# Excalibur-SLE/spmv

Hardware: AMD Instinct MI355X
Metric: fp64 CG iters/sec (SpMV effective GB/s vs HBM roofline) (higher is better)
Workload: dtype f64

## Files before the change

spmv_amd/csrc/hip/common.h:

```cpp
#pragma once

#include <mutex>
#include <vector>

#include <hip/hip_runtime.h>

#include <cstdint>
#include <cstdlib>

#include "spmv_hip.h"

struct spmv_hip_ctx {
  int device = 0;
  int num_cus = 0;
  hipStream_t stream = nullptr;
  int dot_blocks = 0;
  int64_t blas1_nt_min_elems = (int64_t)1 << 24;
  int64_t lx_min_nnz = (int64_t)1 << 20;
  int64_t lx_max_x_bytes = INT64_MAX;
  int lx_dma = 1;
  int lx_codes = 1;
  int lx_narrow_values = 1;
  int lx_ring = 1;
  int release_csr = 0;
  int64_t xw_min_nnz = (int64_t)1 << 20;
  int64_t xw_min_x_bytes = (int64_t)128 << 20;
  int xw_probe = 1;
  int csr_in_place = 0;
  int64_t lat_min_nnz = (int64_t)1 << 20;
  int bake_general = 1;
  int wdia_half = 1;
  int const_diagonals = 1;
  int const_tile = 4;
  int64_t sj_min_nnz = (int64_t)1 << 20;
  int sj_max_chunks = 432;
  int sj_wpb = 0;
  int sj_unit = 0;
  int sj_sigma = 1;
// ... 113 lines not shown
```

spmv_amd/csrc/hip/csr_plan.h:

```cpp
#pragma once

#include "common.h"

#include <chrono>
#include <cstdio>

constexpr int kRows = kBlock;

typedef double f64x2 __attribute__((ext_vector_type(2)));
typedef float f32x4 __attribute__((ext_vector_type(4)));
typedef int i32x2 __attribute__((ext_vector_type(2)));
typedef int i32x4 __attribute__((ext_vector_type(4)));

template <typename T>
struct VecOf;
template <>
struct VecOf<double> {
  static constexpr int V = 2;
  using val_t = f64x2;
  using col_t = i32x2;
};
template <>
struct VecOf<float> {
  static constexpr int V = 4;
// ... 109 lines not shown
}
__host__ __device__ constexpr bool lx_ring_fits(int cnt)
{
  return cnt > 0 && cnt + 3 <= kLxwRingVcap
         && lx_ring_code_bytes(cnt) <= kLxwRingCodeMax;
}
constexpr int kLxwDescStartBits = 11;
constexpr int kLxwDescStartMask = (1 << kLxwDescStartBits) - 1;
constexpr int kLxwDescMaxLen = (1 << (16 - kLxwDescStartBits)) - 1;
static_assert(kLxwRingVcap <= kLxwDescStartMask + 1, "a row's start needs more bits");
constexpr int kLxwDescPad = 1024 - kRows * 2;
__host__ __device__ constexpr int64_t lx_rowdesc_bytes(int64_t num_row_blocks)
{
  return num_row_blocks * (kRows * 2) + kLxwDescPad;
}
constexpr int kXwMaxWin = 8;
constexpr int kXwFirst0 = kLxwPieces0 + kLxwMaxPieces;
constexpr int kXwDelta0 = kXwFirst0 + kXwMaxWin;
constexpr int kXwRec = 36;

constexpr int kLatMaxOff = 8;
constexpr int kLatRec = 12;
constexpr int kWdiaMaxOff = 32;

struct PlanTrace {
  bool on;
  std::chrono::steady_clock::time_point t0;
  const char* who;
  explicit PlanTrace(const char* w)
      : on(getenv("SPMV_PLAN_TRACE") != nullptr), t0(std::chrono::steady_clock::now()),
// ... 183 lines not shown
  int lxw_max_cnt = 0;
  int lxw_max_pieces = 0;
  int lxw_blocks_per_cu = 0;
  int lxw_grid_cap = 0;
  uint8_t* lx_code = nullptr;
  int lx4 = 0;
  int lx4_blocks = 0;
  int lx4_lut = 1;
  int lx_ring_blocks = 0;
  uint16_t* lx_rowdesc = nullptr;
  int lx_ring_pwr = 0;
  int lx_ring = 1;
  float* lx_val32 = nullptr;
  const void* lx32_values0 = nullptr;
  int lx_v32 = 0;
  int32_t* xw_rec = nullptr;
  int xw = 0;
  int xw_staged = 0;
  int xw_max_cnt = 0, xw_max_pieces = 0;
  struct XwProbe* xw_probe = nullptr;
  int32_t* lat_tab = nullptr;
  uint8_t* lat_mask = nullptr;
  int lat = 0;
  int lat_blocks = 0;
  int lat_blocks_per_cu = 4;
  int lat_xcd_group = 0;
  int lat_chain = 1;

  int lattice_d1 = 0, lattice_d2 = 0;

// ... 23 lines not shown
  int use_xw = 1;
  hipEvent_t ev[4][2] = {};
  float us_xw = 0.f, us_gather = 0.f;
};

int spmv_rowblock_grid(const spmv_hip_csr_plan* pl);
bool spmv_released_launch_ok(const spmv_hip_csr_plan* pl, const void* values,
                             const void* in, const void* diagonal, int elem_bytes);
int spmv_build_row_list(spmv_hip_csr_plan* pl, const int32_t* rowptr);
void spmv_free_lx(spmv_hip_csr_plan* pl);
void spmv_free_xw(spmv_hip_csr_plan* pl);
int spmv_build_lx(spmv_hip_csr_plan* pl, const int32_t* rowptr, const int32_t* colind);
int spmv_lx32_bake(spmv_hip_csr_plan* pl, const double* values, bool may_alloc,
                   hipStream_t st);
void spmv_lx32_free(spmv_hip_csr_plan* pl);
int spmv_build_xw_and_walk(spmv_hip_csr_plan* pl, const int32_t* rowptr,
                           const int32_t* colind);
bool spmv_xw_applies(const spmv_hip_csr_plan* pl);
void xw_probe_free(spmv_hip_csr_plan* pl);
void xw_probe_drop_events(XwProbe* pb);
int spmv_plan_owned_mask(const spmv_hip_csr_plan* pl);
int spmv_run_symmetric_f64(const spmv_hip_csr_plan* pl, hipStream_t st,
                           const int32_t* rowptr, const int32_t* colind,
                           const double* values, const double* diagonal,
                           double alpha, const double* in, double beta,
                           double* out, DotOut dot);
int spmv_run_symmetric_f32(const spmv_hip_csr_plan* pl, hipStream_t st,
                           const int32_t* rowptr, const int32_t* colind,
                           const float* values, const float* diagonal,
                           float alpha, const float* in, float beta,
// ... 43 lines not shown
                         double* out, DotOut dot);
int spmv_sdia_run_f64(const spmv_hip_csr_plan* pl, hipStream_t st, double alpha,
                      const double* in, double beta, double* out, DotOut dot);
int spmv_sdia_run_f32(const spmv_hip_csr_plan* pl, hipStream_t st, float alpha,
                      const float* in, float beta, float* out);
int spmv_lxw_grid(const spmv_hip_csr_plan* pl, int elem_bytes);
bool spmv_lxw_ring_ok(const spmv_hip_csr_plan* pl, bool forced);
int spmv_lxw_run_f64(const spmv_hip_csr_plan* pl, hipStream_t st,
                     const int32_t* rowptr, const int32_t* colind,
                     const double* values, double alpha, const double* in,
                     double beta, double* out, DotOut dot);
int spmv_lxw_run_f32f64(const spmv_hip_csr_plan* pl, hipStream_t st,
                        const int32_t* rowptr, const int32_t* colind,
                        const float* values, double alpha, const double* in,
                        double beta, double* out, DotOut dot);
int spmv_xw_grid(const spmv_hip_csr_plan* pl, int elem_bytes);
int spmv_xw_run_f64(const spmv_hip_csr_plan* pl, hipStream_t st,
                    const int32_t* rowptr, const int32_t* colind,
                    const double* values, double alpha, const double* in,
                    double beta, double* out, DotOut dot);
int spmv_xw_run_f32(const spmv_hip_csr_plan* pl, hipStream_t st,
                    const int32_t* rowptr, const int32_t* colind,
                    const float* values, float alpha, const float* in,
                    float beta, float* out);
int spmv_lxw_run_f32(const spmv_hip_csr_plan* pl, hipStream_t st,
                     const int32_t* rowptr, const int32_t* colind,
                     const float* values, float alpha, const float* in,
                     float beta, float* out);
void spmv_wdia_free(spmv_hip_csr_plan* pl);
int spmv_wdia_walk_build(spmv_hip_csr_plan* pl, int segments, bool force);
// ... 56 lines not shown
```

spmv_amd/csrc/hip/runtime.hip:

```cpp
#include "common.h"

#include <cstdio>
#include <cstring>
#include <new>

bool spmv_ctx_watch(spmv_hip_ctx* ctx, const int32_t* word, bool add)
{
  std::lock_guard<std::mutex> lock(ctx->watched_mutex);
  auto& ws = ctx->watched;
  if (add) {
    try {
      ws.push_back(word);
    } catch (...) {
      return false;
    }
    return true;
  }
  for (size_t i = 0; i < ws.size(); ++i)
    if (ws[i] == word) {
      ws[i] = ws.back();
      ws.pop_back();
      break;
    }
  return true;
// ... 131 lines not shown
    *value = ctx->xw_min_nnz;
  else if (!strcmp(key, "xw_min_x_bytes"))
    *value = ctx->xw_min_x_bytes;
  else if (!strcmp(key, "xw_probe"))
    *value = ctx->xw_probe;
  else if (!strcmp(key, "csr_in_place"))
    *value = ctx->csr_in_place;
  else if (!strcmp(key, "lx_min_nnz"))
    *value = ctx->lx_min_nnz;
  else if (!strcmp(key, "lat_min_nnz"))
    *value = ctx->lat_min_nnz;
  else if (!strcmp(key, "lx_narrow_values"))
    *value = ctx->lx_narrow_values;
  else if (!strcmp(key, "lx_ring"))
    *value = ctx->lx_ring;
  else if (!strcmp(key, "sj_min_nnz"))
    *value = ctx->sj_min_nnz;
  else
    return SPMV_HIP_EINVAL;
  return SPMV_HIP_OK;
}

int spmv_hip_ctx_set_option(spmv_hip_ctx* ctx, const char* key, int64_t value)
{
  SPMV_REQUIRE(ctx && key);
  if (!strcmp(key, "blas1_nt_min_elems")) {
    SPMV_REQUIRE(value >= 0);
    ctx->blas1_nt_min_elems = value;
    return SPMV_HIP_OK;
  }
// ... 48 lines not shown
    return SPMV_HIP_OK;
  }
  if (!strcmp(key, "lx_codes")) {
    SPMV_REQUIRE(value == 0 || value == 1);
    ctx->lx_codes = (int)value;
    return SPMV_HIP_OK;
  }
  if (!strcmp(key, "lx_narrow_values")) {
    SPMV_REQUIRE(value == 0 || value == 1);
    ctx->lx_narrow_values = (int)value;
    return SPMV_HIP_OK;
  }
  if (!strcmp(key, "lx_ring")) {
    SPMV_REQUIRE(value >= 0 && value <= 2);
    ctx->lx_ring = (int)value;
    return SPMV_HIP_OK;
  }
  if (!strcmp(key, "poisson_stencil")) {
    SPMV_REQUIRE(value == 7 || value == 27);
    ctx->poisson_stencil = (int)value;
    return SPMV_HIP_OK;
  }
  if (!strcmp(key, "const_diagonals")) {
    SPMV_REQUIRE(value == 0 || value == 1);
    ctx->const_diagonals = (int)value;
    return SPMV_HIP_OK;
  }
  if (!strcmp(key, "const_tile")) {
    SPMV_REQUIRE(value == 1 || value == 2 || value == 4);
    ctx->const_tile = (int)value;
// ... 272 lines not shown
```

spmv_amd/csrc/hip/spmv_csr.hip:

```cpp
#include "csr_plan.h"

#include <cstring>
#include <new>

namespace
{

template <typename TV, typename T, int CH, bool NT, bool ALIGNED, bool DOT,
          bool XCD>
__global__ __launch_bounds__(kBlock) void csr_rowblock_kernel(
    int32_t num_rows, int64_t nnz, const int32_t* __restrict__ rowptr,
    const int32_t* __restrict__ colind, const TV* __restrict__ values, T alpha,
    const T* __restrict__ in, T beta, T* __restrict__ out,
    DotOut dot, RowBlockOrder ord)
{
  constexpr int V = VecOf<TV>::V;
  constexpr int TILE = kBlock * CH * V;
  using val_t = typename VecOf<TV>::val_t;
  using col_t = typename VecOf<TV>::col_t;
  typedef T prod_t __attribute__((ext_vector_type(V)));

  __shared__ __attribute__((aligned(32))) T s_prod[TILE];
  __shared__ int32_t s_rowptr[kRows + 1];
  __shared__ double s_red[kBlock / 64];
// ... 507 lines not shown
    if constexpr (sizeof(T) == 8)
      return spmv_sjds_run_f64(pl, st, alpha, in, beta, out,
                               DOT ? dot : DotOut());
    else
      return spmv_sjds_run_f32(pl, st, alpha, in, beta, out);
  }
  if (pl->lat && aligned16(values)) {
    if constexpr (sizeof(T) == 8)
      return spmv_lat_run_f64(pl, st, rowptr, values, alpha, in, beta, out,
                              DOT ? dot : DotOut());
    else
      return spmv_lat_run_f32(pl, st, rowptr, values, alpha, in, beta, out);
  }
  if (pl->lx && pl->lxw && pl->lxw_rec && al && aligned16(in)) {
    if constexpr (sizeof(T) == 8) {
      if (pl->lx_v32 && pl->lx_val32 && values == pl->lx32_values0)
        return spmv_lxw_run_f32f64(pl, st, rowptr, colind, pl->lx_val32, alpha,
                                   in, beta, out, DOT ? dot : DotOut());
      return spmv_lxw_run_f64(pl, st, rowptr, colind, values, alpha, in, beta,
                              out, DOT ? dot : DotOut());
    } else
      return spmv_lxw_run_f32(pl, st, rowptr, colind, values, alpha, in, beta,
                              out);
  }
  if (pl->lx && al && aligned16(in)) {
    LxView lx{pl->lx_lidx, pl->lx_tab};
    RowBlockOrder lx_ord = pl->row_block_order(nrb);
    if (pl->zwalk && pl->zw_table && pl->zw_grid == grid) {
      lx_ord.table = pl->zw_table;
      lx_ord.num_slots = pl->zw_slots;
// ... 352 lines not shown
```

spmv_amd/csrc/hip/spmv_csr_forms.hip:

```cpp
#include "csr_plan.h"

#include <hipcub/hipcub.hpp>

#include <algorithm>
#include <chrono>
#include <cstring>
#include <new>
#include <utility>
#include <vector>

#include "plan_scratch.h"

namespace
{

template <int ITEMS>
__global__ __launch_bounds__(kBlock) void lx_build_kernel(
    int32_t num_rows, int32_t num_cols, const int32_t* __restrict__ rowptr,
    const int32_t* __restrict__ colind, uint16_t* __restrict__ lidx,
    int32_t* __restrict__ tab, int num_row_blocks, int end_bit, int align,
    int pad, int cap, int32_t* __restrict__ wrec, int32_t* __restrict__ stat,
    int xw)
{
  using Sort = hipcub::BlockRadixSort<int32_t, kBlock, ITEMS, int32_t>;
// ... 334 lines not shown
  pl->num_listed = count;
  return SPMV_HIP_OK;
}

void spmv_free_lx(spmv_hip_csr_plan* pl)
{
  plan_drop(pl->lx_lidx);
  plan_drop(pl->lx_tab);
  plan_drop(pl->lxw_rec);
  plan_drop(pl->lx_code);
  plan_drop(pl->lx_rowdesc);
  pl->lx = pl->lx_staged = pl->lx_blocks = 0;
  pl->lxw = pl->lxw_max_cnt = pl->lxw_max_pieces = 0;
  pl->lx4 = pl->lx4_blocks = pl->lx_ring_blocks = 0;
  spmv_lx32_free(pl);
}

static int build_lx_rowdesc(spmv_hip_csr_plan* pl, const int32_t* rowptr, int nrb,
                            hipStream_t st)
{
  const size_t bytes = (size_t)lx_rowdesc_bytes(nrb);
  hipError_t e = spmv_plan_malloc(&pl->lx_rowdesc, bytes);
  if (e == hipSuccess)
    e = hipMemsetAsync(pl->lx_rowdesc, 0, bytes, st);
  if (e == hipSuccess) {
    int grid = pl->ctx->num_cus * 8;
    grid = grid > nrb ? nrb : grid;
    hipLaunchKernelGGL(lx_rowdesc_kernel, dim3(grid), dim3(kBlock), 0, st,
                       pl->num_rows, rowptr, pl->lxw_rec, pl->lx_rowdesc, nrb);
    e = hipGetLastError();
// ... 144 lines not shown
    e = hipGetLastError();
    if (e == hipSuccess)
      e = hipStreamSynchronize(st);
    if (e == hipSuccess) {
      pl->lx32_values0 = values;
      pl->lx_v32 = 1;
      pl->plan_us += (int)std::chrono::duration_cast<std::chrono::microseconds>(
                         std::chrono::steady_clock::now() - t0)
                         .count();
      return SPMV_HIP_OK;
    }
  }
  spmv_lx32_free(pl);
  if (e == hipErrorOutOfMemory)
    (void)hipGetLastError();
  pl->plan_us += (int)std::chrono::duration_cast<std::chrono::microseconds>(
                     std::chrono::steady_clock::now() - t0)
                     .count();
  return e == hipSuccess || e == hipErrorOutOfMemory ? SPMV_HIP_OK
                                                     : static_cast<int>(e);
}

void spmv_free_xw(spmv_hip_csr_plan* pl)
{
  plan_drop(pl->xw_rec);
  pl->xw = pl->xw_staged = pl->xw_max_cnt = pl->xw_max_pieces = 0;
  xw_probe_free(pl);
}

struct RowBlockEntries {
// ... 405 lines not shown
```

spmv_amd/csrc/hip/spmv_csr_plan.hip:

```cpp
#include "csr_plan.h"

#include <hipcub/hipcub.hpp>

#include <algorithm>
#include <chrono>
#include <cstring>
#include <new>
#include <utility>
#include <vector>

#include "plan_scratch.h"

thread_local int64_t spmv_plan_mem_ns = 0;
thread_local int64_t spmv_plan_live_allocs = 0;

extern "C" int spmv_hip_plan_live_allocations(int64_t* count)
{
  SPMV_REQUIRE(count != nullptr);
  *count = spmv_plan_live_allocs;
  return SPMV_HIP_OK;
}

namespace
{
// ... 82 lines not shown
  SPMV_REQUIRE(ctx && plan && num_rows >= 0 && num_cols >= 0
               && num_non_zeros >= 0);
  SPMV_REQUIRE(num_non_zeros == 0 || (rowptr && colind));
  if (num_non_zeros > 0) {
    SPMV_SET_DEVICE(ctx);
    SPMV_CHECK_HIP(hipStreamSynchronize(spmv_stream(ctx, nullptr)));
  }
  const auto t_begin = std::chrono::steady_clock::now();
  if (num_non_zeros > INT32_MAX)
    return SPMV_HIP_ERANGE;
  spmv_hip_csr_plan* pl = new (std::nothrow) spmv_hip_csr_plan;
  if (!pl)
    return SPMV_HIP_ENOMEM;
  pl->ctx = ctx;
  pl->lx_ring = ctx->lx_ring;
  MemClock mem_clock(pl);
  pl->num_rows = num_rows;
  pl->num_cols = num_cols;
  pl->nnz = num_non_zeros;
  pl->symmetric = symmetric != 0;
  pl->rowptr0 = rowptr;
  pl->colind0 = colind;
  const double avg = num_rows > 0 ? (double)num_non_zeros / num_rows : 0.0;
  if (algo == SPMV_HIP_ALGO_AUTO) {
    if (!symmetric && num_non_zeros > 0 && num_non_zeros * 4 < num_rows)
      algo = SPMV_HIP_ALGO_ROWLIST;
    else
      algo = (avg <= 64.0 || num_non_zeros >= ctx->sj_min_nnz)
                 ? SPMV_HIP_ALGO_ROWBLOCK
                 : SPMV_HIP_ALGO_VECTOR;
// ... 145 lines not shown
        return rx;
      plan->plan_us += (int)std::chrono::duration_cast<std::chrono::microseconds>(
                           std::chrono::steady_clock::now() - t0)
                           .count();
    }
  }
  if (plan->symmetric && (values == nullptr ? plan->sjt != nullptr
                                            : rc == SPMV_HIP_ENOTSUP)) {
    const int rj = sym_sj_bake<double>(ctx, plan, values, diagonal, st);
    rc = values == nullptr ? (rj != SPMV_HIP_OK ? rj : rc) : rj;
  }
  const int rn = spmv_lx32_bake(plan, rc == SPMV_HIP_ENOTSUP ? values : nullptr,
                                !plan->no_new_forms, st);
  if (rn != SPMV_HIP_OK)
    return rn;
  return rc;
}

int spmv_hip_csr_plan_bake_values_f32(spmv_hip_ctx* ctx, spmv_hip_csr_plan* plan,
                                      const float* values, const float* diagonal,
                                      void* stream)
{
  SPMV_SET_DEVICE(ctx);
  SPMV_REQUIRE(plan && plan->ctx == ctx);
  MemClock mem_clock(plan);
  SPMV_REQUIRE(!plan->released);
  hipStream_t st = spmv_stream(ctx, stream);
  if (values)
    SPMV_CHECK_HIP(hipStreamSynchronize(st));
  int rc = spmv_sdia_bake_f32(plan, values, diagonal, st);
// ... 26 lines not shown
      const auto t0 = std::chrono::steady_clock::now();
      const int rx = spmv_build_xw_and_walk(plan, plan->rowptr0, plan->colind0);
      if (rx != SPMV_HIP_OK)
        return rx;
      plan->plan_us += (int)std::chrono::duration_cast<std::chrono::microseconds>(
                           std::chrono::steady_clock::now() - t0)
                           .count();
    }
  }
  if (plan->symmetric && (values == nullptr ? plan->sjt != nullptr
                                            : rc == SPMV_HIP_ENOTSUP)) {
    const int rj = sym_sj_bake<float>(ctx, plan, values, diagonal, st);
    rc = values == nullptr ? (rj != SPMV_HIP_OK ? rj : rc) : rj;
  }
  spmv_lx32_free(plan);
  return rc;
}

int spmv_hip_csr_plan_bake_values_f32f64(spmv_hip_ctx* ctx,
                                         spmv_hip_csr_plan* plan,
                                         const float* values32, void* stream)
{
  SPMV_SET_DEVICE(ctx);
  SPMV_REQUIRE(plan && plan->ctx == ctx);
  MemClock mem_clock(plan);
  SPMV_REQUIRE(!plan->released);
  hipStream_t st = spmv_stream(ctx, stream);
  if (plan->sj_val && !plan->symmetric && !plan->sdia_val && !plan->wdia_val)
    return spmv_sjds_bake_f32f64(plan, values32, st);
  if (plan->wdia_val && !plan->sdia_val)
// ... 46 lines not shown
    if (rc == SPMV_HIP_OK && plan->sj_val32 && plan->sj32_values0)
      rc = spmv_sjds_bake_f32f64(plan, static_cast<const float*>(plan->sj32_values0),
                                 st);
  }
  if (rc == SPMV_HIP_OK && plan->sjt && plan->sjt->sj_val && plan->sjt->sj_values0) {
    const void* v0 = plan->sjt->sj_values0;
    rc = plan->sjt->sj_elem == 8
             ? spmv_sjds_bake_f64(plan->sjt, static_cast<const double*>(v0),
                                  plan->sjv_map, st)
             : spmv_sjds_bake_f32(plan->sjt, static_cast<const float*>(v0),
                                  plan->sjv_map, st);
  }
  if (rc == SPMV_HIP_OK && plan->lx_val32 && plan->lx32_values0)
    rc = spmv_lx32_bake(plan, static_cast<const double*>(plan->lx32_values0), false,
                        st);
  if (rc == SPMV_HIP_OK && (plan->sdia_val || plan->wdia_val)) {
    struct NoNewForms {
      spmv_hip_csr_plan* p;
      ~NoNewForms() { p->no_new_forms = 0; }
    } guard{plan};
    plan->no_new_forms = 1;
    const void* v32 = plan->sdia32_values0 ? plan->sdia32_values0
                                           : plan->wdia32_values0;
    if (plan->sdia_val ? plan->sdia_elem == 8 : plan->wdia_elem == 8) {
      const double* v = static_cast<const double*>(
          plan->sdia_val ? plan->sdia_values0 : plan->wdia_values0);
      const double* d = static_cast<const double*>(plan->sdia_val ? plan->sdia_diag0
                                                                  : nullptr);
      rc = spmv_hip_csr_plan_bake_values_f64(ctx, plan, v, d, stream);
      if (rc == SPMV_HIP_OK && v32) {
// ... 72 lines not shown
    plan->lx = value != 0;
  } else if (!strcmp(key, "lxw")) {
    SPMV_REQUIRE(value == 0 || plan->lxw_rec);
    plan->lxw = value != 0;
    if (plan->zw_table && plan->lx_lidx && !plan->lat_tab)
      return spmv_zwalk_order_build(plan, plan->zw_d2, spmv_walk_grid(plan), 0,
                                    true);
  } else if (!strcmp(key, "lx4")) {
    SPMV_REQUIRE(value == 0 || value == 1);
    SPMV_REQUIRE(value == 0 || plan->lx_code);
    plan->lx4 = value;
  } else if (!strcmp(key, "lx_v32")) {
    SPMV_REQUIRE(value == 0 || value == 1);
    SPMV_REQUIRE(value == 0 || plan->lx_val32);
    plan->lx_v32 = value;
  } else if (!strcmp(key, "lx_ring")) {
    SPMV_REQUIRE(value == 0 || value == 1);
    SPMV_REQUIRE(value == 0 || spmv_lxw_ring_ok(plan, true));
    plan->lx_ring = value ? 2 : 0;
  } else if (!strcmp(key, "lxw_grid_cap")) {
    SPMV_REQUIRE(value >= 0);
    plan->lxw_grid_cap = value;
  } else if (!strcmp(key, "lx_ring_pwr")) {
    SPMV_REQUIRE(value == 0 || value == 3 || value == 4);
    plan->lx_ring_pwr = value == 4 ? 4 : 0;
  } else if (!strcmp(key, "lx4_lut")) {
    SPMV_REQUIRE(value == 1 || value == 2);
    plan->lx4_lut = value;
  } else if (!strcmp(key, "xw")) {
    SPMV_REQUIRE(value == 0 || plan->xw_rec);
// ... 273 lines not shown
    const int64_t n = plan->num_rows, nnz = plan->nnz;
    const int64_t nrb = (n + kRows - 1) / kRows;
    int64_t b = 0;
    if (plan->row_list)
      b += 4 * (int64_t)plan->num_listed;
    if (plan->lx_lidx)
      b += 2 * (nnz + 8) + 4 * nrb * kLxRec;
    if (plan->lxw_rec)
      b += 4 * nrb * kLxwRec;
    if (plan->lx_code)
      b += lx_code_bytes(nnz);
    if (plan->lx_rowdesc)
      b += lx_rowdesc_bytes(nrb);
    if (plan->lx_val32)
      b += 4 * lx32_len(nnz);
    if (plan->xw_rec)
      b += 4 * nrb * kXwRec;
    if (plan->lat_tab)
      b += 48 * nrb + n;
    if (plan->slat_mask)
      b += n;
    const int64_t narr
        = plan->sdia_general == 2 ? 2 * plan->sdia_nd + 1 : plan->sdia_nd + 1;
    if (plan->sdia_val)
      b += narr * plan->sdia_len * plan->sdia_elem + n;
    if (plan->sdia32_val && !plan->sdia_const)
      b += narr * plan->sdia_len * 4 + n;
    if (plan->wdia_val)
      b += (int64_t)plan->wdia_narr * plan->wdia_len * plan->wdia_elem + 4 * n;
    if (plan->wdia32_val && !plan->wdia_const)
// ... 80 lines not shown
    *value = plan->lat_blocks;
  else if (!strcmp(key, "lx"))
    *value = plan->lx;
  else if (!strcmp(key, "lxw"))
    *value = plan->lxw && plan->lxw_rec ? 1 : 0;
  else if (!strcmp(key, "lx4"))
    *value = plan->lx4 && plan->lx_code ? 1 : 0;
  else if (!strcmp(key, "lx4_blocks"))
    *value = plan->lx_code ? plan->lx4_blocks : 0;
  else if (!strcmp(key, "lx4_all"))
    *value = plan->lx_code && plan->lx4_blocks == plan->lx_staged ? 1 : 0;
  else if (!strcmp(key, "lx4_lut"))
    *value = plan->lx4_lut;
  else if (!strcmp(key, "lx_v32"))
    *value = plan->lx_v32 && plan->lx_val32 ? 1 : 0;
  else if (!strcmp(key, "lx_ring"))
    *value = spmv_lxw_ring_ok(plan, false) ? 1 : 0;
  else if (!strcmp(key, "lx_ring_blocks"))
    *value = plan->lx_code ? plan->lx_ring_blocks : 0;
  else if (!strcmp(key, "lxw_grid_cap"))
    *value = plan->lxw_grid_cap;
  else if (!strcmp(key, "lx_ring_pwr"))
    *value = plan->lx_ring_pwr != 4 && plan->lxw_max_pieces <= 12 ? 3 : 4;
  else if (!strcmp(key, "lx_rowdesc"))
    *value = plan->lx_rowdesc ? 1 : 0;
  else if (!strcmp(key, "lxw_grid"))
    *value = plan->lxw_rec ? spmv_lxw_grid(plan, 8) : 0;
  else if (!strcmp(key, "lx_staged"))
    *value = plan->lx_staged;
  else if (!strcmp(key, "lx_blocks"))
// ... 12 lines not shown
```

spmv_amd/csrc/hip/spmv_lxw.hip:

```cpp
#include "csr_plan.h"
#include "lat_dma.h"

#include <new>
#include <type_traits>

namespace
{

struct LxwBlock {
  int rb;
  int nwin;
  int32_t a;
  int32_t cnt;
  int np;
  int own;
  int coded;
};

template <int REC>
__device__ __forceinline__ int32_t lxw_fetch(int rb,
                                             const int32_t* __restrict__ rec)
{
  int32_t w = 0;
  if (rb >= 0) {
// ... 371 lines not shown
               : "memory");
}
template <int N>
__device__ __forceinline__ void ring_wait(double& c, int32_t& d, int32_t& e)
{
  asm volatile("s_waitcnt vmcnt(%3)"
               : "+v"(c), "+v"(d), "+v"(e)
               : "n"(N)
               : "memory");
}

constexpr int kRingDescWave = 2;
constexpr int kRingDumpBytes = 64;
static_assert(lx_ring_code_bytes(kLxwRingVcap - 3) <= kRingDescWave * 1024,
              "a fitting block's codes reach the descriptor wave's piece");
template <bool DOT, bool NT, bool TAB, int VR, int PWR>
__global__ __launch_bounds__(kBlock) void csr_lxw_ring_kernel(
    int32_t num_rows, int32_t num_cols, int64_t nnz,
    const float* __restrict__ values, const uint8_t* __restrict__ code,
    const uint16_t* __restrict__ desc, const int32_t* __restrict__ rec,
    double alpha, const double* __restrict__ in, double beta,
    double* __restrict__ out, DotOut dot, RowBlockOrder ord, int ccap, int xcap)
{
  using T = double;
  constexpr int NW = kBlock / 64;
  constexpr int VCAP = VR * NW * 256;
  constexpr int DMA = VR + 1 + PWR;
  extern __shared__ __attribute__((aligned(16))) unsigned char smem[];
  float* const s_val = reinterpret_cast<float*>(smem);
  unsigned char* const s_code = smem + 3 * (size_t)VCAP * sizeof(float);
  T* const s_x = reinterpret_cast<T*>(s_code + 3 * (size_t)ccap);
  const uint16_t* const s_desc = reinterpret_cast<const uint16_t*>(
      reinterpret_cast<unsigned char*>(s_x) + 3 * (size_t)xcap * sizeof(T));
  __shared__ double s_red[NW];
  __shared__ int32_t s_dict[3 * kLxwDictSize / 2];
  const unsigned lds_val = (unsigned)(uintptr_t)(
      (__attribute__((address_space(3))) void*)s_val);
  const unsigned lds_code = lds_val + 3u * VCAP * (unsigned)sizeof(float);
  const unsigned lds_x = lds_code + 3u * (unsigned)ccap;
  const unsigned lds_desc = lds_x + 3u * (unsigned)xcap * (unsigned)sizeof(T);
  const unsigned lds_dump = lds_desc + 3u * (unsigned)(kRows * 2);

  const int t = threadIdx.x;
  const int wave = __builtin_amdgcn_readfirstlane(t >> 6);
  const int lane = t & 63;
  const int stride = gridDim.x;
  const int num_slots = order_slots(ord);
  double dot_acc = 0.0;
  const int32_t col_last = (num_cols - 2) & ~1;
  const int64_t code_len = lx_code_bytes(nnz);
  const int64_t val_len = lx32_len(nnz);
  const int64_t vdump = lane * 4 < val_len - 4 ? lane * 4 : val_len - 4;
  const int64_t cdump = lane * 16 < code_len - 16 ? lane * 16 : code_len - 16;
  const int32_t xdump = lane * 2 < col_last ? lane * 2 : col_last;

  auto issue = [&](const LxwBlock& b, int32_t w, int sl) {
    const bool live = b.rb >= 0;
    const int64_t a = b.a, e = (int64_t)b.a + b.cnt;
    {
      const int64_t base = a & ~(int64_t)3;
      const int64_t jclamp = (e - 1) & ~(int64_t)3;
      const int pieces = live ? (int)(((e - base) * 4 + 1023) >> 10) : 0;
#pragma unroll
      for (int r = 0; r < VR; ++r) {
        const int q = wave + NW * r;
        const bool real = q < pieces;
        int64_t j = base + (int64_t)(q * 64 + lane) * 4;
        j = j < jclamp ? j : jclamp;
        j = real ? j : vdump;
        if (lane < (real ? 64 : 1))
          glds16<NT>(values + j,
                     real ? lds_val + (unsigned)(sl * VCAP * 4 + q * 1024)
                          : lds_dump);
      }
    }
    {
      const int64_t base = (a >> 1) & ~(int64_t)15, end = (e + 1) >> 1;
      const int64_t jclamp = (end - 1) & ~(int64_t)15;
      const int pieces = live ? (int)((end - base + 1023) >> 10) : 0;
      const bool real = wave < pieces;
      int64_t j = base + (int64_t)(wave * 64 + lane) * 16;
      j = j < jclamp ? j : jclamp;
      j = real ? j : cdump;
      const bool dsc = wave == kRingDescWave;
      const uint8_t* const src
          = dsc ? reinterpret_cast<const uint8_t*>(desc)
                      + (int64_t)(live ? b.rb : 0) * (kRows * 2) + (lane & 31) * 16
                : code + j;
      if (lane < (dsc ? 32 : real ? 64 : 1))
        glds16<NT>(src, dsc ? lds_desc + (unsigned)(sl * (kRows * 2))
                            : real ? lds_code + (unsigned)(sl * ccap + wave * 1024)
                                   : lds_dump);
    }
    const int np = live ? b.np : 0;
#pragma unroll
    for (int k = 0; k < PWR; ++k) {
      const int p = wave + NW * k;
      const bool real = p < np;
      const int32_t col = __builtin_amdgcn_readlane(w, kLxwPieces0 + p);
// ... 62 lines not shown
    const int rb3 = rb_of(it + 3 * stride, raw3);
    int32_t w3 = fetch(rb3);
    int32_t raw4 = raw_of(it + 4 * stride);
    const LxwBlock blk2 = lxw_decode(rb2, w2);
    put_dict(blk2, w2, s2);
    issue(blk2, w2, s2);

    const int32_t r = cur.rb * kRows + t;
    if (cur.rb >= 0 && r < num_rows) {
      T sum = 0;
      T x_own = T(0);
      const int32_t dsc = s_desc[s0 * kRows + t];
      int32_t j = cur.a + (dsc & kLxwDescStartMask);
      const int32_t hi = j + (dsc >> kLxwDescStartBits);
      const float* sv = s_val + (size_t)s0 * VCAP + (cur.a & 3) - cur.a;
      const T* sx = s_x + (size_t)s0 * xcap;
      if constexpr (DOT) {
        if (cur.own >= 0)
          x_own = sx[cur.own + t];
      }
      const uint32_t* sc
          = reinterpret_cast<const uint32_t*>(s_code + (size_t)s0 * ccap);
      const int32_t n0 = cur.a & ~31;
      for (; j < hi; j += 8) {
        const unsigned n = (unsigned)(j - n0);
        const uint32_t c_lo = sc[n >> 3], c_hi = sc[(n >> 3) + 1];
        const uint32_t bits = __builtin_amdgcn_alignbit(c_hi, c_lo, (n & 7) * 4);
        unsigned l[8];
        T v[8], xv[8];
#pragma unroll
        for (int k = 0; k < 8; ++k) {
          const int32_t jj = j + k < hi ? j + k : hi - 1;
          v[k] = (T)sv[jj];
        }
#pragma unroll
        for (int k = 0; k < 8; ++k) {
          const unsigned c = (bits >> (4 * k)) & 15u;
          const int32_t d = reinterpret_cast<const int16_t*>(
              s_dict + s0 * (kLxwDictSize / 2))[c];
          l[k] = j + k < hi ? (unsigned)(t + d) : 0u;
        }
#pragma unroll
        for (int k = 0; k < 8; ++k)
          xv[k] = sx[l[k]];
#pragma unroll
        for (int k = 0; k < 8; ++k)
          if (j + k < hi)
            sum += v[k] * xv[k];
// ... 87 lines not shown
LxwRingGeom lxw_ring_geom(const spmv_hip_csr_plan* pl)
{
  LxwRingGeom g;
  const int max_cnt = pl->lxw_max_cnt < 1 ? 1 : pl->lxw_max_cnt;
  g.ccap = (lx_ring_code_bytes(max_cnt) + 1023) & ~1023;
  int np = pl->lxw_max_pieces;
  np = np < 1 ? 1 : np;
  g.xcap = np * kLxwPiece;
  g.lds = 3 * ((size_t)kLxwRingVcap * sizeof(float) + (size_t)g.ccap
               + (size_t)g.xcap * sizeof(double) + kRows * 2)
          + kRingDumpBytes;
  g.per_cu = (int)((160 * 1024 - 1024) / (g.lds + 256));
  return g;
}

bool lxw_ring_ok(const spmv_hip_csr_plan* pl, bool forced)
{
  const int nrb = (pl->num_rows + kRows - 1) / kRows;
  if (!(forced || pl->lx_ring) || pl->symmetric || !pl->lx || !pl->lxw
      || !pl->lxw_rec || !pl->lx4 || !pl->lx_code || pl->lx4_lut != 1
      || !pl->lx_v32 || !pl->lx_val32 || !pl->lx_rowdesc)
    return false;
  if (nrb < 1 || pl->lx_staged != nrb || pl->lx4_blocks != nrb
      || pl->lx_ring_blocks != nrb || !lx_ring_fits(pl->lxw_max_cnt)
      || pl->lxw_max_pieces > kLxwMaxPieces)
    return false;
  if (lxw_ring_geom(pl).per_cu < lxw_geom(pl, 8, 2).per_cu)
    return false;
  constexpr int kMinSteps = 128;
  const int grid = lxw_grid(pl, 8, 2);
  return forced || pl->lx_ring >= 2 || (nrb + grid - 1) / grid >= kMinSteps;
}

template <bool DOT, int PWR>
int lxw_ring_launch_p(const spmv_hip_csr_plan* pl, hipStream_t st,
                      const float* values, double alpha, const double* in,
                      double beta, double* out, DotOut dot)
{
  constexpr int VR = kLxwRingValRounds;
  const LxwRingGeom g = lxw_ring_geom(pl);
  const int nrb = (pl->num_rows + kRows - 1) / kRows;
  const int grid = lxw_grid(pl, 8, 2);
  RowBlockOrder ord = pl->row_block_order(nrb);
  ord.xcd_group = pl->lat_xcd_group;
  if (pl->zwalk && pl->zw_table && pl->zw_grid == grid) {
    ord.table = pl->zw_table;
    ord.num_slots = pl->zw_slots;
  }
  auto kern
      = ord.table
            ? (pl->nontemporal ? csr_lxw_ring_kernel<DOT, true, true, VR, PWR>
                               : csr_lxw_ring_kernel<DOT, false, true, VR, PWR>)
            : (pl->nontemporal ? csr_lxw_ring_kernel<DOT, true, false, VR, PWR>
                               : csr_lxw_ring_kernel<DOT, false, false, VR, PWR>);
  if (g.lds > 48 * 1024)
    SPMV_CHECK_HIP(hipFuncSetAttribute(
        reinterpret_cast<const void*>(kern),
        hipFuncAttributeMaxDynamicSharedMemorySize, (int)g.lds));
  hipLaunchKernelGGL(kern, dim3(grid), dim3(kBlock), g.lds, st, pl->num_rows,
                     pl->num_cols, pl->nnz, values, pl->lx_code, pl->lx_rowdesc,
                     pl->lxw_rec, alpha, in, beta, out, dot, ord, g.ccap, g.xcap);
  SPMV_CHECK_LAUNCH();
  return SPMV_HIP_OK;
}

template <bool DOT>
int lxw_ring_launch(const spmv_hip_csr_plan* pl, hipStream_t st,
                    const float* values, double alpha, const double* in,
                    double beta, double* out, DotOut dot)
{
  constexpr int NW = kBlock / 64, PWR = kLxwMaxPieces / NW;
  if (pl->lx_ring_pwr != PWR && pl->lxw_max_pieces <= (PWR - 1) * NW)
    return lxw_ring_launch_p<DOT, PWR - 1>(pl, st, values, alpha, in, beta, out,
                                           dot);
  return lxw_ring_launch_p<DOT, PWR>(pl, st, values, alpha, in, beta, out, dot);
}

template <typename TV, typename T, bool DOT, bool XW, int C4>
int lxw_launch_c(const spmv_hip_csr_plan* pl, hipStream_t st,
                 const int32_t* rowptr, const int32_t* colind, const TV* values,
                 T alpha, const T* in, T beta, T* out, DotOut dot)
{
  const LxwGeom g = lxw_geom(pl, (int)sizeof(T), XW ? 4 : 2);
  const int vcap = g.vcap * (int)(sizeof(T) / sizeof(TV));
  const int nrb = (pl->num_rows + kRows - 1) / kRows;
  const int grid = lxw_grid(pl, (int)sizeof(T), XW ? 4 : 2);
  RowBlockOrder ord = pl->row_block_order(nrb);
  ord.xcd_group = pl->lat_xcd_group;
  if (pl->zwalk && pl->zw_table && pl->zw_grid == grid) {
    ord.table = pl->zw_table;
// ... 14 lines not shown
                     XW ? nullptr : pl->lx_lidx, C4 ? pl->lx_code : nullptr,
                     XW ? pl->xw_rec : pl->lxw_rec, alpha, in, beta, out, dot,
                     ord, vcap, g.lcap, g.xcap);
  SPMV_CHECK_LAUNCH();
  return SPMV_HIP_OK;
}

template <typename TV, typename T, bool DOT, bool XW>
int lxw_launch(const spmv_hip_csr_plan* pl, hipStream_t st,
               const int32_t* rowptr, const int32_t* colind, const TV* values,
               T alpha, const T* in, T beta, T* out, DotOut dot)
{
  if constexpr (!XW && std::is_same<TV, float>::value
                && std::is_same<T, double>::value) {
    if (lxw_ring_ok(pl, false))
      return lxw_ring_launch<DOT>(pl, st, values, alpha, in, beta, out, dot);
  }
  if constexpr (!XW) {
    if (pl->lx4 && pl->lx_code)
      return pl->lx4_lut == 2
                 ? lxw_launch_c<TV, T, DOT, XW, 2>(pl, st, rowptr, colind, values,
                                                   alpha, in, beta, out, dot)
                 : lxw_launch_c<TV, T, DOT, XW, 1>(pl, st, rowptr, colind, values,
                                                   alpha, in, beta, out, dot);
  }
  return lxw_launch_c<TV, T, DOT, XW, 0>(pl, st, rowptr, colind, values, alpha,
                                         in, beta, out, dot);
}

}

int spmv_lxw_grid(const spmv_hip_csr_plan* pl, int elem_bytes)
{
  return lxw_grid(pl, elem_bytes, 2);
}

bool spmv_lxw_ring_ok(const spmv_hip_csr_plan* pl, bool forced)
{
  return lxw_ring_ok(pl, forced);
}

int spmv_xw_grid(const spmv_hip_csr_plan* pl, int elem_bytes)
{
  return lxw_grid(pl, elem_bytes, 4);
}

int spmv_lxw_run_f64(const spmv_hip_csr_plan* pl, hipStream_t st,
                     const int32_t* rowptr, const int32_t* colind,
                     const double* values, double alpha, const double* in,
                     double beta, double* out, DotOut dot)
{
  if (dot.partials)
    return lxw_launch<double, double, true, false>(pl, st, rowptr, colind, values,
                                                   alpha, in, beta, out, dot);
  return lxw_launch<double, double, false, false>(pl, st, rowptr, colind, values,
                                                  alpha, in, beta, out, dot);
// ... 44 lines not shown
```

Baseline: 335.0.

## Encode CSR values as 4-bit per-block dictionary codes in the ring kernel

Adds a plan-time encoder that, for each row block with at most 16 distinct values, stores a 16-entry fp64 dictionary and a 4-bit code per nonzero. The ring SpMV kernel gains a VC variant that DMA-loads these codes and the dictionary into LDS instead of fp32 values, then decodes by table lookup. This is meant to cut value-stream HBM traffic from 4 bytes to half a byte per nonzero while keeping values exact in fp64. The cost is extra plan-time encoding and LDS lookups, and the path only activates when every block fits in 16 distinct values.

```diff
diff --git a/spmv_amd/csrc/hip/common.h b/spmv_amd/csrc/hip/common.h
--- a/spmv_amd/csrc/hip/common.h
+++ b/spmv_amd/csrc/hip/common.h
@@ -22,6 +22,7 @@
   int lx_codes = 1;
   int lx_narrow_values = 1;
   int lx_ring = 1;
+  int lx_vcode = 1;
   int release_csr = 0;
   int64_t xw_min_nnz = (int64_t)1 << 20;
   int64_t xw_min_x_bytes = (int64_t)128 << 20;
diff --git a/spmv_amd/csrc/hip/csr_plan.h b/spmv_amd/csrc/hip/csr_plan.h
--- a/spmv_amd/csrc/hip/csr_plan.h
+++ b/spmv_amd/csrc/hip/csr_plan.h
@@ -147,6 +147,7 @@
 {
   return num_row_blocks * (kRows * 2) + kLxwDescPad;
 }
+constexpr int kLxVcDictSize = 16;
 constexpr int kXwMaxWin = 8;
 constexpr int kXwFirst0 = kLxwPieces0 + kLxwMaxPieces;
 constexpr int kXwDelta0 = kXwFirst0 + kXwMaxWin;
@@ -360,6 +361,11 @@
   float* lx_val32 = nullptr;
   const void* lx32_values0 = nullptr;
   int lx_v32 = 0;
+  uint8_t* lx_vcode = nullptr;
+  double* lx_vdict = nullptr;
+  const void* lx_vc_values0 = nullptr;
+  int lx_vcode_blocks = 0;
+  int lx_vc = 1;
   int32_t* xw_rec = nullptr;
   int xw = 0;
   int xw_staged = 0;
@@ -413,6 +419,9 @@
 int spmv_lx32_bake(spmv_hip_csr_plan* pl, const double* values, bool may_alloc,
                    hipStream_t st);
 void spmv_lx32_free(spmv_hip_csr_plan* pl);
+int spmv_lxvc_bake(spmv_hip_csr_plan* pl, const int32_t* rowptr,
+                   const double* values, bool may_alloc, hipStream_t st);
+void spmv_lxvc_free(spmv_hip_csr_plan* pl);
 int spmv_build_xw_and_walk(spmv_hip_csr_plan* pl, const int32_t* rowptr,
                            const int32_t* colind);
 bool spmv_xw_applies(const spmv_hip_csr_plan* pl);
@@ -486,6 +495,9 @@
                         const int32_t* rowptr, const int32_t* colind,
                         const float* values, double alpha, const double* in,
                         double beta, double* out, DotOut dot);
+bool spmv_lxw_vcode_ok(const spmv_hip_csr_plan* pl);
+int spmv_lxw_run_vcode(const spmv_hip_csr_plan* pl, hipStream_t st, double alpha,
+                       const double* in, double beta, double* out, DotOut dot);
 int spmv_xw_grid(const spmv_hip_csr_plan* pl, int elem_bytes);
 int spmv_xw_run_f64(const spmv_hip_csr_plan* pl, hipStream_t st,
                     const int32_t* rowptr, const int32_t* colind,
diff --git a/spmv_amd/csrc/hip/runtime.hip b/spmv_amd/csrc/hip/runtime.hip
--- a/spmv_amd/csrc/hip/runtime.hip
+++ b/spmv_amd/csrc/hip/runtime.hip
@@ -169,6 +169,8 @@
     *value = ctx->lx_narrow_values;
   else if (!strcmp(key, "lx_ring"))
     *value = ctx->lx_ring;
+  else if (!strcmp(key, "lx_vcode"))
+    *value = ctx->lx_vcode;
   else if (!strcmp(key, "sj_min_nnz"))
     *value = ctx->sj_min_nnz;
   else
@@ -247,6 +249,11 @@
   if (!strcmp(key, "lx_ring")) {
     SPMV_REQUIRE(value >= 0 && value <= 2);
     ctx->lx_ring = (int)value;
+    return SPMV_HIP_OK;
+  }
+  if (!strcmp(key, "lx_vcode")) {
+    SPMV_REQUIRE(value == 0 || value == 1);
+    ctx->lx_vcode = (int)value;
     return SPMV_HIP_OK;
   }
   if (!strcmp(key, "poisson_stencil")) {
diff --git a/spmv_amd/csrc/hip/spmv_csr.hip b/spmv_amd/csrc/hip/spmv_csr.hip
--- a/spmv_amd/csrc/hip/spmv_csr.hip
+++ b/spmv_amd/csrc/hip/spmv_csr.hip
@@ -545,6 +545,9 @@
   }
   if (pl->lx && pl->lxw && pl->lxw_rec && al && aligned16(in)) {
     if constexpr (sizeof(T) == 8) {
+      if (values == pl->lx_vc_values0 && spmv_lxw_vcode_ok(pl))
+        return spmv_lxw_run_vcode(pl, st, alpha, in, beta, out,
+                                  DOT ? dot : DotOut());
       if (pl->lx_v32 && pl->lx_val32 && values == pl->lx32_values0)
         return spmv_lxw_run_f32f64(pl, st, rowptr, colind, pl->lx_val32, alpha,
                                    in, beta, out, DOT ? dot : DotOut());
diff --git a/spmv_amd/csrc/hip/spmv_csr_forms.hip b/spmv_amd/csrc/hip/spmv_csr_forms.hip
--- a/spmv_amd/csrc/hip/spmv_csr_forms.hip
+++ b/spmv_amd/csrc/hip/spmv_csr_forms.hip
@@ -372,6 +372,7 @@
   pl->lxw = pl->lxw_max_cnt = pl->lxw_max_pieces = 0;
   pl->lx4 = pl->lx4_blocks = pl->lx_ring_blocks = 0;
   spmv_lx32_free(pl);
+  spmv_lxvc_free(pl);
 }
 
 static int build_lx_rowdesc(spmv_hip_csr_plan* pl, const int32_t* rowptr, int nrb,
@@ -546,6 +547,183 @@
   spmv_lx32_free(pl);
   if (e == hipErrorOutOfMemory)
     (void)hipGetLastError();
+  pl->plan_us += (int)std::chrono::duration_cast<std::chrono::microseconds>(
+                     std::chrono::steady_clock::now() - t0)
+                     .count();
+  return e == hipSuccess || e == hipErrorOutOfMemory ? SPMV_HIP_OK
+                                                     : static_cast<int>(e);
+}
+
+namespace
+{
+
+__global__ __launch_bounds__(kBlock) void lxvc_encode_kernel(
+    int32_t num_rows, const int32_t* __restrict__ rowptr,
+    const double* __restrict__ values, const int32_t* __restrict__ wrec,
+    uint32_t* __restrict__ code, double* __restrict__ dict, int num_row_blocks,
+    int32_t* __restrict__ stat)
+{
+  constexpr int CAP = kBlock * 16;
+  __shared__ unsigned long long s_dict[kLxVcDictSize];
+  __shared__ unsigned long long s_min;
+  __shared__ int s_any;
+  __shared__ uint32_t s_pack[CAP / 8 + 2];
+  const int t = threadIdx.x;
+  const unsigned long long* bits
+      = reinterpret_cast<const unsigned long long*>(values);
+  int coded = 0;
+  for (int rb = blockIdx.x; rb < num_row_blocks; rb += gridDim.x) {
+    const int32_t* wr = wrec + (int64_t)rb * kLxwRec;
+    const int32_t a = wr[1], cnt = wr[2];
+    const int nwin = wr[0];
+    __syncthreads();
+    if (nwin < 0 || cnt <= 0 || cnt > CAP)
+      continue;
+    const int32_t a0 = a & ~7;
+    const int nwords = (int)(((int64_t)a + cnt + 7 - a0) >> 3);
+    for (int w = t; w < nwords; w += kBlock)
+      s_pack[w] = 0;
+    if (t < kLxVcDictSize)
+      s_dict[t] = 0;
+    const int32_t r = rb * kRows + t;
+    int32_t lo = 0, hi = 0;
+    if (r < num_rows) {
+      lo = rowptr[r];
+      hi = rowptr[r + 1];
+    }
+    int n = 0;
+    bool more = false;
+    unsigned long long last = 0;
+    for (int k = 0; k <= kLxVcDictSize; ++k) {
+      if (t == 0) {
+        s_min = ~0ull;
+        s_any = 0;
+      }
+      __syncthreads();
+      bool have = false;
+      unsigned long long m = ~0ull;
+      for (int32_t j = lo; j < hi; ++j) {
+        const unsigned long long b = bits[j];
+        if ((k == 0 || b > last) && (!have || b < m)) {
+          m = b;
+          have = true;
+        }
+      }
+      if (have) {
+        atomicMin(&s_min, m);
+        s_any = 1;
+      }
+      __syncthreads();
+      const bool any = s_any != 0;
+      last = s_min;
+      __syncthreads();
+      if (!any)
+        break;
+      if (k == kLxVcDictSize) {
+        more = true;
+        break;
+      }
+      if (t == 0)
+        s_dict[k] = last;
+      n = k + 1;
+    }
+    if (more)
+      continue;
+    __syncthreads();
+    for (int32_t j = lo; j < hi; ++j) {
+      const unsigned long long b = bits[j];
+      uint32_t c = 0;
+      for (int k = 1; k < n; ++k)
+        c += s_dict[k] <= b ? 1u : 0u;
+      const int q = j - a0;
+      atomicOr(&s_pack[q >> 3], c << ((q & 7) * 4));
+    }
+    __syncthreads();
+    for (int w = t; w < nwords; w += kBlock) {
+      const bool whole = (w > 0 || a0 == a) && (int64_t)a0 + 8 * (w + 1) <= (int64_t)a + cnt;
+      uint32_t* dst = code + ((int64_t)a0 >> 3) + w;
+      if (whole)
+        *dst = s_pack[w];
+      else if (s_pack[w])
+        atomicOr(dst, s_pack[w]);
+    }
+    if (t < kLxVcDictSize)
+      reinterpret_cast<unsigned long long*>(dict)[(int64_t)rb * kLxVcDictSize + t]
+          = s_dict[t];
+    if (t == 0)
+      ++coded;
+  }
+  if (t == 0 && coded)
+    atomicAdd(&stat[0], coded);
+}
+
+}
+
+void spmv_lxvc_free(spmv_hip_csr_plan* pl)
+{
+  plan_drop(pl->lx_vcode);
+  plan_drop(pl->lx_vdict);
+  pl->lx_vc_values0 = nullptr;
+  pl->lx_vcode_blocks = 0;
+}
+
+int spmv_lxvc_bake(spmv_hip_csr_plan* pl, const int32_t* rowptr,
+                   const double* values, bool may_alloc, hipStream_t st)
+{
+  const int nrb = (pl->num_rows + kRows - 1) / kRows;
+  if (!values || !rowptr || pl->symmetric || !(pl->lx && pl->lxw && pl->lxw_rec)
+      || !pl->ctx->lx_vcode || pl->nnz == 0 || !aligned16(values) || !pl->lx_code
+      || !pl->lx_rowdesc || nrb < 1 || pl->lx_staged != nrb
+      || pl->lx4_blocks != nrb || pl->lx_ring_blocks != nrb
+      || pl->lxw_max_pieces > kLxwMaxPieces) {
+    spmv_lxvc_free(pl);
+    return SPMV_HIP_OK;
+  }
+  const auto t0 = std::chrono::steady_clock::now();
+  const size_t code_bytes = (size_t)lx_code_bytes(pl->nnz);
+  const size_t dict_bytes = sizeof(double) * kLxVcDictSize * (size_t)nrb;
+  hipError_t e = hipSuccess;
+  if (!(pl->lx_vcode && pl->lx_vdict)) {
+    spmv_lxvc_free(pl);
+    e = may_alloc ? spmv_plan_malloc(&pl->lx_vcode, code_bytes)
+                  : hipErrorOutOfMemory;
+    if (e != hipSuccess)
+      pl->lx_vcode = nullptr;
+    else if ((e = spmv_plan_malloc(&pl->lx_vdict, dict_bytes)) != hipSuccess)
+      pl->lx_vdict = nullptr;
+  }
+  PlanScratch<int32_t> d_stat;
+  int32_t h_stat = 0;
+  if (e == hipSuccess)
+    e = d_stat.alloc(1);
+  if (e == hipSuccess)
+    e = hipMemsetAsync(pl->lx_vcode, 0, code_bytes, st);
+  if (e == hipSuccess)
+    e = hipMemsetAsync(pl->lx_vdict, 0, dict_bytes, st);
+  if (e == hipSuccess)
+    e = hipMemsetAsync(d_stat.get(), 0, sizeof(int32_t), st);
+  if (e == hipSuccess) {
+    int grid = pl->ctx->num_cus * 8;
+    grid = grid > nrb ? nrb : grid;
+    hipLaunchKernelGGL(lxvc_encode_kernel, dim3(grid), dim3(kBlock), 0, st,
+                       pl->num_rows, rowptr, values, pl->lxw_rec,
+                       reinterpret_cast<uint32_t*>(pl->lx_vcode), pl->lx_vdict,
+                       nrb, d_stat.get());
+    e = hipGetLastError();
+  }
+  if (e == hipSuccess)
+    e = plan_fetch(&h_stat, d_stat.get(), 1, st);
+  d_stat.reset();
+  if (e == hipSuccess && h_stat == nrb) {
+    pl->lx_vc_values0 = values;
+    pl->lx_vcode_blocks = h_stat;
+  } else {
+    spmv_lxvc_free(pl);
+    if (e == hipSuccess)
+      pl->lx_vcode_blocks = h_stat;
+    else
+      (void)hipGetLastError();
+  }
   pl->plan_us += (int)std::chrono::duration_cast<std::chrono::microseconds>(
                      std::chrono::steady_clock::now() - t0)
                      .count();
diff --git a/spmv_amd/csrc/hip/spmv_csr_plan.hip b/spmv_amd/csrc/hip/spmv_csr_plan.hip
--- a/spmv_amd/csrc/hip/spmv_csr_plan.hip
+++ b/spmv_amd/csrc/hip/spmv_csr_plan.hip
@@ -120,6 +120,7 @@
     return SPMV_HIP_ENOMEM;
   pl->ctx = ctx;
   pl->lx_ring = ctx->lx_ring;
+  pl->lx_vc = ctx->lx_vcode;
   MemClock mem_clock(pl);
   pl->num_rows = num_rows;
   pl->num_cols = num_cols;
@@ -295,6 +296,11 @@
                                 !plan->no_new_forms, st);
   if (rn != SPMV_HIP_OK)
     return rn;
+  const int rv = spmv_lxvc_bake(plan, plan->rowptr0,
+                                rc == SPMV_HIP_ENOTSUP ? values : nullptr,
+                                !plan->no_new_forms, st);
+  if (rv != SPMV_HIP_OK)
+    return rv;
   return rc;
 }
 
@@ -351,6 +357,7 @@
     rc = values == nullptr ? (rj != SPMV_HIP_OK ? rj : rc) : rj;
   }
   spmv_lx32_free(plan);
+  spmv_lxvc_free(plan);
   return rc;
 }
 
@@ -427,6 +434,9 @@
   if (rc == SPMV_HIP_OK && plan->lx_val32 && plan->lx32_values0)
     rc = spmv_lx32_bake(plan, static_cast<const double*>(plan->lx32_values0), false,
                         st);
+  if (rc == SPMV_HIP_OK && plan->lx_vcode && plan->lx_vc_values0)
+    rc = spmv_lxvc_bake(plan, plan->rowptr0,
+                        static_cast<const double*>(plan->lx_vc_values0), false, st);
   if (rc == SPMV_HIP_OK && (plan->sdia_val || plan->wdia_val)) {
     struct NoNewForms {
       spmv_hip_csr_plan* p;
@@ -529,6 +539,9 @@
     SPMV_REQUIRE(value == 0 || value == 1);
     SPMV_REQUIRE(value == 0 || plan->lx_val32);
     plan->lx_v32 = value;
+  } else if (!strcmp(key, "lx_vcode")) {
+    SPMV_REQUIRE(value == 0 || value == 1);
+    plan->lx_vc = value;
   } else if (!strcmp(key, "lx_ring")) {
     SPMV_REQUIRE(value == 0 || value == 1);
     SPMV_REQUIRE(value == 0 || spmv_lxw_ring_ok(plan, true));
@@ -832,6 +845,10 @@
       b += lx_rowdesc_bytes(nrb);
     if (plan->lx_val32)
       b += 4 * lx32_len(nnz);
+    if (plan->lx_vcode)
+      b += lx_code_bytes(nnz);
+    if (plan->lx_vdict)
+      b += 8 * kLxVcDictSize * nrb;
     if (plan->xw_rec)
       b += 4 * nrb * kXwRec;
     if (plan->lat_tab)
@@ -942,6 +959,15 @@
     *value = plan->lx4_lut;
   else if (!strcmp(key, "lx_v32"))
     *value = plan->lx_v32 && plan->lx_val32 ? 1 : 0;
+  else if (!strcmp(key, "lx_vcode"))
+    *value = plan->lx_vc && plan->lx_vcode && plan->lx_vdict ? 1 : 0;
+  else if (!strcmp(key, "lx_vcode_blocks"))
+    *value = plan->lx_vcode_blocks;
+  else if (!strcmp(key, "lx_vcode_all"))
+    *value = plan->lx_vcode && plan->lx_vdict
+                     && plan->lx_vcode_blocks == (plan->num_rows + kRows - 1) / kRows
+                 ? 1
+                 : 0;
   else if (!strcmp(key, "lx_ring"))
     *value = spmv_lxw_ring_ok(plan, false) ? 1 : 0;
   else if (!strcmp(key, "lx_ring_blocks"))
diff --git a/spmv_amd/csrc/hip/spmv_lxw.hip b/spmv_amd/csrc/hip/spmv_lxw.hip
--- a/spmv_amd/csrc/hip/spmv_lxw.hip
+++ b/spmv_amd/csrc/hip/spmv_lxw.hip
@@ -409,21 +409,29 @@
 constexpr int kRingDumpBytes = 64;
 static_assert(lx_ring_code_bytes(kLxwRingVcap - 3) <= kRingDescWave * 1024,
               "a fitting block's codes reach the descriptor wave's piece");
-template <bool DOT, bool NT, bool TAB, int VR, int PWR>
+template <bool DOT, bool NT, bool TAB, int VR, int PWR, bool VC>
 __global__ __launch_bounds__(kBlock) void csr_lxw_ring_kernel(
     int32_t num_rows, int32_t num_cols, int64_t nnz,
-    const float* __restrict__ values, const uint8_t* __restrict__ code,
+    const float* __restrict__ values, const uint8_t* __restrict__ vcode,
+    const double* __restrict__ vdict, const uint8_t* __restrict__ code,
     const uint16_t* __restrict__ desc, const int32_t* __restrict__ rec,
     double alpha, const double* __restrict__ in, double beta,
     double* __restrict__ out, DotOut dot, RowBlockOrder ord, int ccap, int xcap)
 {
   using T = double;
+  static_assert(!VC || VR == 1, "value codes: one value piece per wave");
   constexpr int NW = kBlock / 64;
   constexpr int VCAP = VR * NW * 256;
   constexpr int DMA = VR + 1 + PWR;
+  constexpr int DB = kLxVcDictSize * (int)sizeof(double);
   extern __shared__ __attribute__((aligned(16))) unsigned char smem[];
+  const unsigned val_bytes
+      = VC ? 3u * ((unsigned)ccap + DB) : 3u * VCAP * (unsigned)sizeof(float);
   float* const s_val = reinterpret_cast<float*>(smem);
-  unsigned char* const s_code = smem + 3 * (size_t)VCAP * sizeof(float);
+  const unsigned char* const s_vcode = smem;
+  const double* const s_vdict
+      = reinterpret_cast<const double*>(smem + 3 * (size_t)ccap);
+  unsigned char* const s_code = smem + val_bytes;
   T* const s_x = reinterpret_cast<T*>(s_code + 3 * (size_t)ccap);
   const uint16_t* const s_desc = reinterpret_cast<const uint16_t*>(
       reinterpret_cast<unsigned char*>(s_x) + 3 * (size_t)xcap * sizeof(T));
@@ -431,7 +439,8 @@
   __shared__ int32_t s_dict[3 * kLxwDictSize / 2];
   const unsigned lds_val = (unsigned)(uintptr_t)(
       (__attribute__((address_space(3))) void*)s_val);
-  const unsigned lds_code = lds_val + 3u * VCAP * (unsigned)sizeof(float);
+  const unsigned lds_vdict = lds_val + 3u * (unsigned)ccap;
+  const unsigned lds_code = lds_val + val_bytes;
   const unsigned lds_x = lds_code + 3u * (unsigned)ccap;
   const unsigned lds_desc = lds_x + 3u * (unsigned)xcap * (unsigned)sizeof(T);
   const unsigned lds_dump = lds_desc + 3u * (unsigned)(kRows * 2);
@@ -452,7 +461,7 @@
   auto issue = [&](const LxwBlock& b, int32_t w, int sl) {
     const bool live = b.rb >= 0;
     const int64_t a = b.a, e = (int64_t)b.a + b.cnt;
-    {
+    if constexpr (!VC) {
       const int64_t base = a & ~(int64_t)3;
       const int64_t jclamp = (e - 1) & ~(int64_t)3;
       const int pieces = live ? (int)(((e - base) * 4 + 1023) >> 10) : 0;
@@ -478,6 +487,17 @@
       j = j < jclamp ? j : jclamp;
       j = real ? j : cdump;
       const bool dsc = wave == kRingDescWave;
+      if constexpr (VC) {
+        const uint8_t* const vsrc
+            = dsc ? reinterpret_cast<const uint8_t*>(
+                        vdict + (int64_t)(live ? b.rb : 0) * kLxVcDictSize)
+                        + (lane & 7) * 16
+                  : vcode + j;
+        if (lane < (dsc ? DB / 16 : real ? 64 : 1))
+          glds16<NT>(vsrc, dsc ? lds_vdict + (unsigned)(sl * DB)
+                               : real ? lds_val + (unsigned)(sl * ccap + wave * 1024)
+                                      : lds_dump);
+      }
       const uint8_t* const src
           = dsc ? reinterpret_cast<const uint8_t*>(desc)
                       + (int64_t)(live ? b.rb : 0) * (kRows * 2) + (lane & 31) * 16
@@ -570,6 +590,9 @@
       int32_t j = cur.a + (dsc & kLxwDescStartMask);
       const int32_t hi = j + (dsc >> kLxwDescStartBits);
       const float* sv = s_val + (size_t)s0 * VCAP + (cur.a & 3) - cur.a;
+      const uint32_t* svc
+          = reinterpret_cast<const uint32_t*>(s_vcode + (size_t)s0 * ccap);
+      const T* sd = s_vdict + s0 * kLxVcDictSize;
       const T* sx = s_x + (size_t)s0 * xcap;
       if constexpr (DOT) {
         if (cur.own >= 0)
@@ -584,10 +607,19 @@
         const uint32_t bits = __builtin_amdgcn_alignbit(c_hi, c_lo, (n & 7) * 4);
         unsigned l[8];
         T v[8], xv[8];
-#pragma unroll
-        for (int k = 0; k < 8; ++k) {
-          const int32_t jj = j + k < hi ? j + k : hi - 1;
-          v[k] = (T)sv[jj];
+        if constexpr (VC) {
+          const uint32_t v_lo = svc[n >> 3], v_hi = svc[(n >> 3) + 1];
+          const uint32_t vbits
+              = __builtin_amdgcn_alignbit(v_hi, v_lo, (n & 7) * 4);
+#pragma unroll
+          for (int k = 0; k < 8; ++k)
+            v[k] = sd[(vbits >> (4 * k)) & 15u];
+        } else {
+#pragma unroll
+          for (int k = 0; k < 8; ++k) {
+            const int32_t jj = j + k < hi ? j + k : hi - 1;
+            v[k] = (T)sv[jj];
+          }
         }
 #pragma unroll
         for (int k = 0; k < 8; ++k) {
@@ -705,12 +737,19 @@
   return g;
 }
 
+bool lxw_vcode_on(const spmv_hip_csr_plan* pl)
+{
+  const int nrb = (pl->num_rows + kRows - 1) / kRows;
+  return pl->lx_vc && pl->lx_vcode && pl->lx_vdict && pl->lx_vc_values0
+         && pl->lx_vcode_blocks == nrb;
+}
+
 bool lxw_ring_ok(const spmv_hip_csr_plan* pl, bool forced)
 {
   const int nrb = (pl->num_rows + kRows - 1) / kRows;
   if (!(forced || pl->lx_ring) || pl->symmetric || !pl->lx || !pl->lxw
       || !pl->lxw_rec || !pl->lx4 || !pl->lx_code || pl->lx4_lut != 1
-      || !pl->lx_v32 || !pl->lx_val32 || !pl->lx_rowdesc)
+      || !((pl->lx_v32 && pl->lx_val32) || lxw_vcode_on(pl)) || !pl->lx_rowdesc)
     return false;
   if (nrb < 1 || pl->lx_staged != nrb || pl->lx4_blocks != nrb
       || pl->lx_ring_blocks != nrb || !lx_ring_fits(pl->lxw_max_cnt)
@@ -723,12 +762,12 @@
   return forced || pl->lx_ring >= 2 || (nrb + grid - 1) / grid >= kMinSteps;
 }
 
-template <bool DOT, int PWR>
+template <bool DOT, int PWR, bool VC>
 int lxw_ring_launch_p(const spmv_hip_csr_plan* pl, hipStream_t st,
                       const float* values, double alpha, const double* in,
                       double beta, double* out, DotOut dot)
 {
-  constexpr int VR = kLxwRingValRounds;
+  constexpr int VR = VC ? 1 : kLxwRingValRounds;
   const LxwRingGeom g = lxw_ring_geom(pl);
   const int nrb = (pl->num_rows + kRows - 1) / kRows;
   const int grid = lxw_grid(pl, 8, 2);
@@ -740,31 +779,33 @@
   }
   auto kern
       = ord.table
-            ? (pl->nontemporal ? csr_lxw_ring_kernel<DOT, true, true, VR, PWR>
-                               : csr_lxw_ring_kernel<DOT, false, true, VR, PWR>)
-            : (pl->nontemporal ? csr_lxw_ring_kernel<DOT, true, false, VR, PWR>
-                               : csr_lxw_ring_kernel<DOT, false, false, VR, PWR>);
+            ? (pl->nontemporal ? csr_lxw_ring_kernel<DOT, true, true, VR, PWR, VC>
+                               : csr_lxw_ring_kernel<DOT, false, true, VR, PWR, VC>)
+            : (pl->nontemporal ? csr_lxw_ring_kernel<DOT, true, false, VR, PWR, VC>
+                               : csr_lxw_ring_kernel<DOT, false, false, VR, PWR, VC>);
   if (g.lds > 48 * 1024)
     SPMV_CHECK_HIP(hipFuncSetAttribute(
         reinterpret_cast<const void*>(kern),
         hipFuncAttributeMaxDynamicSharedMemorySize, (int)g.lds));
   hipLaunchKernelGGL(kern, dim3(grid), dim3(kBlock), g.lds, st, pl->num_rows,
-                     pl->num_cols, pl->nnz, values, pl->lx_code, pl->lx_rowdesc,
-                     pl->lxw_rec, alpha, in, beta, out, dot, ord, g.ccap, g.xcap);
+                     pl->num_cols, pl->nnz, values, pl->lx_vcode, pl->lx_vdict,
+                     pl->lx_code, pl->lx_rowdesc, pl->lxw_rec, alpha, in, beta, out,
+                     dot, ord, g.ccap, g.xcap);
   SPMV_CHECK_LAUNCH();
   return SPMV_HIP_OK;
 }
 
-template <bool DOT>
+template <bool DOT, bool VC>
 int lxw_ring_launch(const spmv_hip_csr_plan* pl, hipStream_t st,
                     const float* values, double alpha, const double* in,
                     double beta, double* out, DotOut dot)
 {
   constexpr int NW = kBlock / 64, PWR = kLxwMaxPieces / NW;
   if (pl->lx_ring_pwr != PWR && pl->lxw_max_pieces <= (PWR - 1) * NW)
-    return lxw_ring_launch_p<DOT, PWR - 1>(pl, st, values, alpha, in, beta, out,
-                                           dot);
-  return lxw_ring_launch_p<DOT, PWR>(pl, st, values, alpha, in, beta, out, dot);
+    return lxw_ring_launch_p<DOT, PWR - 1, VC>(pl, st, values, alpha, in, beta,
+                                               out, dot);
+  return lxw_ring_launch_p<DOT, PWR, VC>(pl, st, values, alpha, in, beta, out,
+                                         dot);
 }
 
 template <typename TV, typename T, bool DOT, bool XW, int C4>
@@ -809,7 +850,8 @@
   if constexpr (!XW && std::is_same<TV, float>::value
                 && std::is_same<T, double>::value) {
     if (lxw_ring_ok(pl, false))
-      return lxw_ring_launch<DOT>(pl, st, values, alpha, in, beta, out, dot);
+      return lxw_ring_launch<DOT, false>(pl, st, values, alpha, in, beta, out,
+                                         dot);
   }
   if constexpr (!XW) {
     if (pl->lx4 && pl->lx_code)
@@ -835,6 +877,19 @@
   return lxw_ring_ok(pl, forced);
 }
 
+bool spmv_lxw_vcode_ok(const spmv_hip_csr_plan* pl)
+{
+  return lxw_vcode_on(pl) && lxw_ring_ok(pl, false);
+}
+
+int spmv_lxw_run_vcode(const spmv_hip_csr_plan* pl, hipStream_t st, double alpha,
+                       const double* in, double beta, double* out, DotOut dot)
+{
+  if (dot.partials)
+    return lxw_ring_launch<true, true>(pl, st, nullptr, alpha, in, beta, out, dot);
+  return lxw_ring_launch<false, true>(pl, st, nullptr, alpha, in, beta, out, dot);
+}
+
 int spmv_xw_grid(const spmv_hip_csr_plan* pl, int elem_bytes)
 {
   return lxw_grid(pl, elem_bytes, 4);
```

New measurement: 349.9 (median of 6 runs). 1.04x the previous value.
